# zhiyuan-yang/MILE

Hardware: AMD Instinct MI355X
Metric: MCLMC integrator particle-steps/s (integrator-steps/s x ensemble size) (higher is better)
Workload: dtype f32

## Files before the change

include/mile_hip.h:

```cpp
#ifndef MILE_HIP_H_
#define MILE_HIP_H_

#include <stdint.h>

#ifdef __cplusplus
extern "C" {
#endif

#define MILE_ABI_VERSION 6
#define MILE_MAX_LAYERS 16

typedef enum mile_status {
  MILE_OK = 0,
  MILE_ERR_INVALID = -1,
  MILE_ERR_STATE = -2,
  MILE_ERR_HIP = -3,
  MILE_ERR_NOMEM = -4
} mile_status;

typedef enum mile_activation { MILE_ACT_RELU = 0, MILE_ACT_TANH = 1, MILE_ACT_SIGMOID = 2 } mile_activation;
typedef enum mile_task { MILE_TASK_REGRESSION = 0, MILE_TASK_CLASSIFICATION = 1 } mile_task;
typedef enum mile_prior { MILE_PRIOR_NORMAL = 0, MILE_PRIOR_LAPLACE = 1 } mile_prior;
typedef enum mile_refresh { MILE_REFRESH_O_STEP_O = 0, MILE_REFRESH_STEP_O = 1 } mile_refresh;
typedef enum mile_grad_kernel {
  MILE_GRAD_AUTO = 0,
  MILE_GRAD_GENERIC = 1,
  MILE_GRAD_MFMA_W64 = 2,
  MILE_GRAD_MFMA_W128_BF16 = 3,
  MILE_GRAD_GEMM_F32 = 4,
  MILE_GRAD_LENET_F32 = 5,
  MILE_GRAD_MFMA_W64_BF16X3 = 6,
  MILE_GRAD_MFMA_WIDE_BF16X3 = 7,
  MILE_GRAD_MFMA_WIDE_BF16 = 8,
  MILE_GRAD_MFMA_NARROW_F32 = 10,
  MILE_GRAD_LENET_BF16 = 9,
  MILE_GRAD_LENETTI_F32 = 11
} mile_grad_kernel;
typedef enum mile_model { MILE_MODEL_FCN = 0, MILE_MODEL_LENET = 1, MILE_MODEL_LENETTI = 2 } mile_model;

typedef struct mile_model_spec {
  int32_t in_features;
  int32_t n_layers;
// ... 112 lines not shown

int32_t mile_set_row_window(mile_sampler *s, int64_t begin, int64_t count);

int32_t mile_warmstart_step(mile_sampler *s, float *theta, int32_t E, const mile_optim_args *args, void *stream);

int32_t mile_reserve(mile_sampler *s, int32_t E);

int32_t mile_set_grad_kernel(mile_sampler *s, int32_t which);
int32_t mile_get_grad_kernel(const mile_sampler *s);

int32_t mile_logpost_grad(mile_sampler *s, const float *theta, int32_t E, float *logp, float *grad,
                          void *stream);

int32_t mile_init(mile_sampler *s, mile_state *state, const float *noise, uint64_t seed,
                  const int32_t *particle_ids, void *stream);

int32_t mile_step(mile_sampler *s, mile_state *state, const mile_step_args *args, void *stream);

int32_t mile_tune(mile_sampler *s, mile_state *state, const mile_tune_args *args, void *stream);

int32_t mile_pointwise_loglik(mile_sampler *s, const float *theta, int32_t S, const float *X, const void *y,
                              int64_t N, float *out, void *stream);

int32_t mile_nuts_reserve(mile_sampler *s, int32_t E, int32_t max_num_doublings);

int32_t mile_nuts_step(mile_sampler *s, mile_state *state, const mile_nuts_args *a, void *stream);

int32_t mile_nuts_warmup(mile_sampler *s, mile_state *state, const mile_nuts_args *a, const mile_nuts_adapt_args *w,
                         void *stream);

int32_t mile_debug_noise(mile_sampler *s, uint64_t seed, const int32_t *particle_ids, int32_t E,
                         int64_t step, int32_t stage, float *out, void *stream);

int32_t mile_grad_launch_info(const mile_sampler *s, int32_t E, int32_t *grid_x, int32_t *grid_y,
                              int32_t *block, int32_t *lds_bytes, char *name, int32_t name_len);

int32_t mile_grad_timing_begin(mile_sampler *s);
int32_t mile_grad_timing_end(mile_sampler *s, float *total_ms, int32_t *n_launches);

#ifdef __cplusplus
}
#endif
#endif
```

mile_amd/_lib.py:

```python
from __future__ import annotations

import ctypes as C
from pathlib import Path

from mile_amd._build import LIB_PATH

MILE_MAX_LAYERS = 16
ABI_VERSION = 6

ACTIVATION_IDS = {'relu': 0, 'tanh': 1, 'sigmoid': 2}
TASK_IDS = {'regr': 0, 'regression': 0, 'classification': 1, 'class': 1}
PRIOR_IDS = {'Normal': 0, 'StandardNormal': 0, 'Laplace': 1}
REFRESH_IDS = {'O-step-O': 0, 'step-O': 1}
GRAD_KERNEL_IDS = {'auto': 0, 'generic': 1, 'mfma_w64': 2, 'mfma_w128_bf16': 3, 'gemm_f32': 4, 'lenet_f32': 5, 'mfma_w64_bf16x3': 6,
                   'mfma_wide_bf16x3': 7, 'mfma_wide_bf16': 8, 'lenet_bf16': 9, 'mfma_narrow_f32': 10,
                   'lenetti_f32': 11}


class ModelSpecC(C.Structure):
    _fields_ = [
        ('in_features', C.c_int32),
        ('n_layers', C.c_int32),
        ('widths', C.c_int32 * MILE_MAX_LAYERS),
        ('activation', C.c_int32),
        ('task', C.c_int32),
        ('prior', C.c_int32),
        ('prior_loc', C.c_float),
        ('prior_scale', C.c_float),
        ('use_bias', C.c_int32),
        ('model', C.c_int32),
        ('img_c', C.c_int32),
        ('img_h', C.c_int32),
        ('img_w', C.c_int32),
    ]


class StateC(C.Structure):
    _fields_ = [
        ('n_particles', C.c_int32),
        ('position', C.c_void_p),
        ('momentum', C.c_void_p),
# ... 50 lines not shown
        ('seed', C.c_uint64), ('particle_ids', C.c_void_p), ('step_offset', C.c_int64), ('n_steps', C.c_int32),
        ('n_thinning', C.c_int32), ('out_samples', C.c_void_p), ('out_info', C.c_void_p),
        ('out_stats', C.POINTER(C.c_int64)),
    ]


class NutsAdaptArgsC(C.Structure):
    _fields_ = [
        ('step_size', C.c_void_p), ('inverse_mass_matrix', C.c_void_p), ('da', C.c_void_p), ('welford', C.c_void_p),
        ('welford_count', C.c_void_p), ('schedule', C.POINTER(C.c_int32)), ('target_acceptance_rate', C.c_float),
    ]

SIGNATURES = {
    'mile_last_error': (C.c_char_p, []),
    'mile_abi_version': (C.c_int32, []),
    'mile_create': (C.c_int32, [C.POINTER(ModelSpecC), C.c_int32, C.POINTER(C.c_void_p)]),
    'mile_destroy': (C.c_int32, [C.c_void_p]),
    'mile_param_count': (C.c_int64, [C.c_void_p]),
    'mile_param_offsets': (C.c_int32, [C.c_void_p, C.c_int32, C.POINTER(C.c_int64), C.POINTER(C.c_int64)]),
    'mile_set_data': (C.c_int32, [C.c_void_p, C.c_void_p, C.c_void_p, C.c_int64, C.c_void_p]),
    'mile_set_row_window': (C.c_int32, [C.c_void_p, C.c_int64, C.c_int64]),
    'mile_reserve': (C.c_int32, [C.c_void_p, C.c_int32]),
    'mile_warmstart_step': (C.c_int32, [C.c_void_p, C.c_void_p, C.c_int32, C.POINTER(OptimArgsC), C.c_void_p]),
    'mile_set_grad_kernel': (C.c_int32, [C.c_void_p, C.c_int32]),
    'mile_get_grad_kernel': (C.c_int32, [C.c_void_p]),
    'mile_logpost_grad': (C.c_int32, [C.c_void_p, C.c_void_p, C.c_int32, C.c_void_p, C.c_void_p, C.c_void_p]),
    'mile_init': (C.c_int32, [C.c_void_p, C.POINTER(StateC), C.c_void_p, C.c_uint64, C.c_void_p, C.c_void_p]),
    'mile_step': (C.c_int32, [C.c_void_p, C.POINTER(StateC), C.POINTER(StepArgsC), C.c_void_p]),
    'mile_tune': (C.c_int32, [C.c_void_p, C.POINTER(StateC), C.POINTER(TuneArgsC), C.c_void_p]),
    'mile_pointwise_loglik': (C.c_int32, [C.c_void_p, C.c_void_p, C.c_int32, C.c_void_p, C.c_void_p, C.c_int64,
                                          C.c_void_p, C.c_void_p]),
    'mile_debug_noise': (C.c_int32, [C.c_void_p, C.c_uint64, C.c_void_p, C.c_int32, C.c_int64, C.c_int32,
                                     C.c_void_p, C.c_void_p]),
    'mile_grad_launch_info': (C.c_int32, [C.c_void_p, C.c_int32, C.POINTER(C.c_int32), C.POINTER(C.c_int32),
                                          C.POINTER(C.c_int32), C.POINTER(C.c_int32), C.c_char_p, C.c_int32]),
    'mile_nuts_reserve': (C.c_int32, [C.c_void_p, C.c_int32, C.c_int32]),
    'mile_nuts_step': (C.c_int32, [C.c_void_p, C.POINTER(StateC), C.POINTER(NutsArgsC), C.c_void_p]),
    'mile_nuts_warmup': (C.c_int32, [C.c_void_p, C.POINTER(StateC), C.POINTER(NutsArgsC), C.POINTER(NutsAdaptArgsC),
                                     C.c_void_p]),
    'mile_grad_timing_begin': (C.c_int32, [C.c_void_p]),
    'mile_grad_timing_end': (C.c_int32, [C.c_void_p, C.POINTER(C.c_float), C.POINTER(C.c_int32)]),
}

_lib = None


class MileHipError(RuntimeError):
    pass


def load_library(path: str | Path | None = None) -> C.CDLL:
    global _lib
    if _lib is not None and path is None:
        return _lib
    p = Path(path) if path else LIB_PATH
    if not p.exists():
        raise MileHipError(
            f'{p} not found: the MI355X HIP extension is not built. Run '
            '`python -c "import __graft_entry__ as g; g.build()"` (needs hipcc). '
            'mile_amd has no CPU fallback.')
    try:
        lib = C.CDLL(str(p))
    except OSError as exc:
        raise MileHipError(f'cannot load {p}: {exc}') from exc
    for name, (res, args) in SIGNATURES.items():
        try:
# ... 18 lines not shown
```

mile_amd/csrc/mile_hip.hip:

```cpp
#include <hip/hip_runtime.h>

#include <algorithm>
#include <cmath>
#include <cstdio>
#include <cstdlib>
#include <cstring>
#include <string>
#include <vector>

#include <dlfcn.h>

#include "mile_device.h"
#include "mile_grad_generic.h"
#include "mile_grad_narrow.h"
#include "mile_grad_w64.h"
#include "mile_grad_w128b.h"
#include "mile_grad_gemm.h"
#include "mile_mm3.h"
#include "mile_lenet.h"
#include "mile_lenet_mfma.h"
#include "mile_lenetti.h"
#include "mile_predict.h"
#include "mile_update.h"
#include "mile_nuts.h"

static thread_local std::string g_err;
static int fail(int code, const std::string &msg) { g_err = msg; return code; }
#define HIP_TRY(expr)                                                                         \
  do {                                                                                        \
    hipError_t _e = (expr);                                                                   \
    if (_e != hipSuccess)                                                                     \
      return fail(MILE_ERR_HIP, std::string(#expr) + ": " + hipGetErrorString(_e));           \
  } while (0)

static const double MCLACHLAN_B1 = 0.1931833275037836;

struct mile_sampler {
  mile_model_spec spec{};
  DevSpec ds{};
  int device = 0;
  int n_cu = 256;
  float *X = nullptr, *Xp = nullptr;
  void *Xb = nullptr, *Xt = nullptr;
  void *y = nullptr;
  int N = 0, Npad = 0, Fp = 0, Npb = 0;
  int win_begin = 0, win_count = 0;
  int E_cap = 0;
  size_t ES_cap = 0;
  float *slabs = nullptr, *llpart = nullptr, *dK = nullptr, *lold = nullptr;
  float *upart = nullptr;
  int32_t *arrive = nullptr;
  float *ev_X = nullptr, *ev_Xp = nullptr; void *ev_y = nullptr; int ev_cap = 0;
  float *alt_x = nullptr, *alt_u = nullptr, *alt_g = nullptr, *alt_logp = nullptr;
  int grad_kernel = MILE_GRAD_AUTO;
  LeNetGeom lg{};
  LeNettiGeom ng{};
  void *blas = nullptr;
  long long *dbg_buf = nullptr;
  float *tune_info = nullptr;
  float *gemm_ws = nullptr, *gemm_ones = nullptr;
  int gemm_ones_n = 0;
  size_t gemm_ws_floats = 0;
  int gemm_R = 0, gemm_E = 0;
  float *wide_ws = nullptr; size_t wide_ws_floats = 0; int wide_R = 0, wide_E = 0;
  void *wide_wt = nullptr; size_t wide_wt_bytes = 0;
  float *wide_hb = nullptr; size_t wide_hb_floats = 0;
  NutsBufs nb{};
  int nuts_E = 0, nuts_M = 0;
  int32_t *nuts_count_h = nullptr;
  bool timing = false;
  std::vector<hipEvent_t> ev;
  size_t ev_used = 0;
};

static bool w64_supported(const mile_model_spec &sp) {
  if (sp.model != MILE_MODEL_FCN) return false;
  if (sp.task != MILE_TASK_REGRESSION || sp.activation != MILE_ACT_RELU) return false;
  const int nh = sp.n_layers - 1;
  if (nh < 1 || nh > 3) return false;
  for (int l = 0; l < nh; ++l)
    if (sp.widths[l] != 64) return false;
  if (sp.widths[nh] != 2) return false;
  if (sp.in_features > 16) return false;
  return true;
// ... 256 lines not shown
  hipError_t e = hipGetDeviceCount(&cnt);
  if (e == hipSuccess && device < cnt) {
    hipDeviceProp_t prop;
    if (hipGetDeviceProperties(&prop, device) == hipSuccess) s->n_cu = prop.multiProcessorCount;
  }
  *out = s;
  return MILE_OK;
}

static void free_data(mile_sampler *s) {
  if (s->X) (void)hipFree(s->X);
  if (s->Xp) (void)hipFree(s->Xp);
  if (s->y) (void)hipFree(s->y);
  if (s->Xb) (void)hipFree(s->Xb);
  if (s->Xt) (void)hipFree(s->Xt);
  s->X = s->Xp = nullptr; s->y = nullptr; s->Xb = s->Xt = nullptr;
}
static void free_ws(mile_sampler *s) {
  if (s->slabs) (void)hipFree(s->slabs);
  if (s->llpart) (void)hipFree(s->llpart);
  if (s->dK) (void)hipFree(s->dK);
  if (s->upart) (void)hipFree(s->upart);
  s->upart = nullptr;
  if (s->lold) (void)hipFree(s->lold);
  if (s->alt_x) (void)hipFree(s->alt_x);
  if (s->alt_u) (void)hipFree(s->alt_u);
  if (s->alt_g) (void)hipFree(s->alt_g);
  if (s->alt_logp) (void)hipFree(s->alt_logp);
  s->alt_x = s->alt_u = s->alt_g = s->alt_logp = nullptr;
  if (s->tune_info) (void)hipFree(s->tune_info);
  s->tune_info = nullptr;
  if (s->arrive) (void)hipFree(s->arrive);
  s->arrive = nullptr;
  if (s->dbg_buf) (void)hipFree(s->dbg_buf);
  s->dbg_buf = nullptr;
  s->slabs = s->llpart = s->dK = s->lold = nullptr;
  s->E_cap = 0; s->ES_cap = 0;
}

static void free_nuts(mile_sampler *s) {
  NutsBufs &b = s->nb;
  float **fs[] = {&b.T, &b.Ph, &b.xe[0], &b.xe[1], &b.pe[0], &b.pe[1], &b.ge[0], &b.ge[1], &b.psT, &b.psS, &b.xs, &b.gs,
                  &b.ck_r, &b.ck_rs};
  for (float **f : fs) { if (*f) (void)hipFree(*f); *f = nullptr; }
  if (b.chain) (void)hipFree(b.chain);
  if (b.count) (void)hipFree(b.count);
  b.chain = nullptr; b.count = nullptr;
  s->nuts_E = s->nuts_M = 0;
}

int32_t mile_destroy(mile_sampler *s) {
  if (!s) return MILE_OK;
  if (s->ev_X) (void)hipFree(s->ev_X);
  if (s->ev_Xp) (void)hipFree(s->ev_Xp);
  if (s->ev_y) (void)hipFree(s->ev_y);
  free_data(s);
  free_ws(s);
  if (s->gemm_ws) (void)hipFree(s->gemm_ws);
  if (s->gemm_ones) (void)hipFree(s->gemm_ones);
  if (s->wide_ws) (void)hipFree(s->wide_ws);
  if (s->wide_wt) (void)hipFree(s->wide_wt);
  if (s->wide_hb) (void)hipFree(s->wide_hb);
  if (s->dbg_buf) (void)hipFree(s->dbg_buf);
  if (s->tune_info) (void)hipFree(s->tune_info);
  free_nuts(s);
  if (s->nuts_count_h) (void)hipHostFree(s->nuts_count_h);
// ... 62 lines not shown
    HIP_TRY(hipMalloc(&s->X, (size_t)N * F * 4));
    HIP_TRY(hipMalloc(&s->Xp, (size_t)(s->Npad + 32) * s->Fp * 4));
    HIP_TRY(hipMalloc(&s->y, (size_t)(s->Npad + 32) * 4));
  }
  HIP_TRY(hipMemsetAsync(s->Xp, 0, (size_t)(s->Npad + 32) * s->Fp * 4, st));
  HIP_TRY(hipMemcpyAsync(s->X, X, (size_t)N * F * 4, hipMemcpyDeviceToDevice, st));
  HIP_TRY(hipMemsetAsync(s->y, 0, (size_t)(s->Npad + 32) * 4, st));
  s->win_begin = s->win_count = 0;
  HIP_TRY(hipMemcpyAsync(s->y, y, (size_t)N * 4, hipMemcpyDeviceToDevice, st));
  const long long tot = (long long)s->Npad * s->Fp;
  k_pad_x<<<(unsigned)((tot + 255) / 256), 256, 0, st>>>(s->X, s->Xp, s->N, s->Npad, F, s->Fp);
  HIP_TRY(hipGetLastError());
  if (w128b_supported(s->spec)) {
    s->Npb = ((int)N + 63) / 64 * 64;
    if (!same_shape) {
      HIP_TRY(hipMalloc(&s->Xb, (size_t)s->Npb * 16 * 2));
      HIP_TRY(hipMalloc(&s->Xt, (size_t)s->Npb * 32 * 2));
    }
    const long long tb = (long long)s->Npb * 32;
    k_prep_bf16<<<(unsigned)((tb + 255) / 256), 256, 0, st>>>(s->X, (bf16 *)s->Xb, (bf16 *)s->Xt, s->N, s->Npb, F);
    HIP_TRY(hipGetLastError());
  }
  return MILE_OK;
}

int32_t mile_set_row_window(mile_sampler *s, int64_t begin, int64_t count) {
  if (!s) return fail(MILE_ERR_INVALID, "null handle");
  if (!s->X) return fail(MILE_ERR_STATE, "mile_set_row_window: call mile_set_data first");
  if (begin < 0 || count < 0 || begin + count > s->N) return fail(MILE_ERR_INVALID, "mile_set_row_window: window outside the data");
  s->win_begin = count ? (int)begin : 0;
  s->win_count = (int)count;
  return MILE_OK;
}

int32_t mile_reserve(mile_sampler *s, int32_t E) {
  if (!s || E < 1) return fail(MILE_ERR_INVALID, "mile_reserve: bad argument");
  if (!s->X) return fail(MILE_ERR_STATE, "mile_reserve: call mile_set_data first");
  HIP_TRY(hipSetDevice(s->device));
  int S = std::max(choose_S(s, E, MILE_GRAD_GENERIC), w64_supported(s->spec) ? choose_S(s, E, MILE_GRAD_MFMA_W64) : 1);
  if (w128b_supported(s->spec)) S = std::max(S, choose_S(s, E, MILE_GRAD_MFMA_W128_BF16));
  if (narrow_supported(s->spec)) S = std::max(S, choose_S(s, E, MILE_GRAD_MFMA_NARROW_F32));
  if (s->spec.model == MILE_MODEL_LENETTI) S = std::max(S, choose_S(s, E, MILE_GRAD_LENETTI_F32));
  if (E <= s->E_cap && (size_t)E * S <= s->ES_cap) return MILE_OK;
  const int En = std::max(E, s->E_cap);
  const size_t ESn = std::max((size_t)E * S, s->ES_cap);
  free_ws(s);
  HIP_TRY(hipMalloc(&s->slabs, ESn * ((s->ds.d + 3) / 4 * 4) * 4));
  HIP_TRY(hipMalloc(&s->llpart, ESn * 4));
  HIP_TRY(hipMalloc(&s->dK, (size_t)En * 4));
  HIP_TRY(hipMalloc(&s->lold, (size_t)En * 4));
  HIP_TRY(hipMalloc(&s->upart, ((size_t)En * ((s->ds.d + UPD_SEG - 1) / UPD_SEG) * UPD_NSUM + (size_t)En * 8) * 4));
  HIP_TRY(hipMalloc(&s->alt_x, (size_t)En * s->ds.d * 4));
  HIP_TRY(hipMalloc(&s->alt_u, (size_t)En * s->ds.d * 4));
  HIP_TRY(hipMalloc(&s->alt_g, (size_t)En * s->ds.d * 4));
  HIP_TRY(hipMalloc(&s->alt_logp, (size_t)En * 4));
  HIP_TRY(hipMalloc(&s->arrive, ((size_t)En * 4 + 15) / 16 * 16));
  HIP_TRY(hipMemset(s->arrive, 0, ((size_t)En * 4 + 15) / 16 * 16));
  s->E_cap = En;
  s->ES_cap = ESn;
  return MILE_OK;
}

int32_t mile_set_grad_kernel(mile_sampler *s, int32_t which) {
  if (!s) return fail(MILE_ERR_INVALID, "null handle");
  if (which < MILE_GRAD_AUTO || which > MILE_GRAD_LENETTI_F32) return fail(MILE_ERR_INVALID, "unknown grad kernel");
  if ((s->spec.model == MILE_MODEL_LENETTI) != (which == MILE_GRAD_LENETTI_F32) && which != MILE_GRAD_AUTO)
    return fail(MILE_ERR_INVALID, "LENETTI_F32 is the kernel of MILE_MODEL_LENETTI, and its only one");
  if (which == MILE_GRAD_MFMA_NARROW_F32 && !narrow_supported(s->spec))
    return fail(MILE_ERR_INVALID, "MFMA_NARROW_F32 needs an FCN with 1-3 hidden layers of width <= 64 and F <= 64 (or 4-10 of width <= 16 and F <= 16) and <= 16 outputs");
  if ((which == MILE_GRAD_MFMA_WIDE_BF16X3 || which == MILE_GRAD_MFMA_WIDE_BF16) && s->spec.model != MILE_MODEL_FCN)
    return fail(MILE_ERR_INVALID, "MFMA_WIDE_* are FCN kernels");
  if ((s->spec.model == MILE_MODEL_LENET) != (which == MILE_GRAD_LENET_F32 || which == MILE_GRAD_LENET_BF16) && which != MILE_GRAD_AUTO)
    return fail(MILE_ERR_INVALID, "LENET_F32 / LENET_BF16 are the kernels of MILE_MODEL_LENET, and its only ones");
  if (which == MILE_GRAD_LENET_BF16 && s->lg.C > 4) return fail(MILE_ERR_INVALID, "LENET_BF16 needs <= 4 image channels");
  if (which == MILE_GRAD_GEMM_F32 && !rocblas_load()) return fail(MILE_ERR_HIP, "GEMM_F32 needs librocblas.so, which could not be loaded");
  if (which == MILE_GRAD_MFMA_W128_BF16 && !w128b_supported(s->spec))
    return fail(MILE_ERR_INVALID, "MFMA_W128_BF16 needs ReLU regression with 1-3 hidden layers of width 128 and F <= 16");
  if (which == MILE_GRAD_MFMA_W64 && !w64_supported(s->spec))
    return fail(MILE_ERR_INVALID, "MFMA_W64 needs ReLU regression with 1-3 hidden layers of width 64 and F <= 16");
  if (which == MILE_GRAD_MFMA_W64_BF16X3 && !w64x3_supported(s->spec))
    return fail(MILE_ERR_INVALID, "MFMA_W64_BF16X3 needs ReLU regression with 2-3 hidden layers of width 64 and F <= 16");
  s->grad_kernel = which;
  return MILE_OK;
}
int32_t mile_get_grad_kernel(const mile_sampler *s) { return s ? resolved_kernel(s) : MILE_ERR_INVALID; }

}

static int ptr_align(const void *q) {
  const uintptr_t a = (uintptr_t)q;
  return (a & 15) == 0 ? 4 : ((a & 7) == 0 ? 2 : 1);
}

template <int AL, bool SDC>
static void launch_update_al(const UpdParams &u, int E, int nk, hipStream_t st) {
  const int nqf = u.d >> 2;
  const int nt = std::min(UPD_NT, ((nqf + nk - 1) / nk + 63) / 64 * 64);
  const int kind = SDC ? -1 : upd_kind(u);
#define MILE_UPD_CASE(NK_)                                                                       \
  if constexpr (!SDC) {                                                                          \
    if (kind == UPD_KIND_MID) { k_update_fast<NK_, AL, SDC, UPD_KIND_MID><<<E, nt, 0, st>>>(u); break; } \
    if (kind == UPD_KIND_REC) { k_update_fast<NK_, AL, SDC, UPD_KIND_REC><<<E, nt, 0, st>>>(u); break; } \
    if (kind == UPD_KIND_TUNE) {                                                                 \
      if (nt <= 768) k_update_fast<NK_, AL, SDC, UPD_KIND_TUNE, 768><<<E, nt, 0, st>>>(u);       \
      else k_update_fast<NK_, AL, SDC, UPD_KIND_TUNE><<<E, nt, 0, st>>>(u);                      \
      break;                                                                                     \
    }                                                                                            \
  }                                                                                              \
  if (nt <= 768) k_update_fast<NK_, AL, SDC, -1, 768><<<E, nt, 0, st>>>(u);                      \
  else k_update_fast<NK_, AL, SDC><<<E, nt, 0, st>>>(u);                                         \
  break;
  switch (nk) {
    case 1: MILE_UPD_CASE(1)
    case 2: MILE_UPD_CASE(2)
    case 3: MILE_UPD_CASE(3)
    default: MILE_UPD_CASE(4)
  }
#undef MILE_UPD_CASE
}

template <int AL, bool SDC>
static bool launch_update_big_al(const UpdParams &u, int E, int nk, hipStream_t st) {
  const int nqf = u.d >> 2;
  const int nt = std::min(UPD_NT, ((nqf + nk - 1) / nk + 63) / 64 * 64);
  const size_t lds = (size_t)nk * nt * 16;
#define MILE_UPD_BIG(NK_, CF_)                                                                                     \
  {                                                                                                                \
    static bool attr = false;                                                                                      \
    if (!attr) {                                                                                                   \
      if (hipFuncSetAttribute((const void *)k_update_big<NK_, AL, SDC, CF_>, hipFuncAttributeMaxDynamicSharedMemorySize, \
                              UPD_NT * NK_ * 16) != hipSuccess) return false;                                      \
      attr = true;                                                                                                 \
    }                                                                                                              \
    k_update_big<NK_, AL, SDC, CF_><<<E, nt, lds, st>>>(u);                                                        \
    return true;                                                                                                   \
  }
#define MILE_UPD_BIG_CASE(NK_) \
  case NK_:                    \
    MILE_UPD_BIG(NK_, -1)
  switch (nk) {
    MILE_UPD_BIG_CASE(5)
    MILE_UPD_BIG_CASE(6)
    MILE_UPD_BIG_CASE(7)
    MILE_UPD_BIG_CASE(8)
    MILE_UPD_BIG_CASE(9)
  }
#undef MILE_UPD_BIG_CASE
#undef MILE_UPD_BIG
  return false;
}

static bool launch_update_big(const UpdParams &u, int E, hipStream_t st) {
  const int nqf = u.d >> 2;
  const int nk = (nqf + UPD_NT - 1) / UPD_NT;
  if (nk <= UPD_QMAX || nk > UPD_QMAX_BIG || (u.flags & UPD_TUNE) || u.zA || u.zB || getenv("MILE_NO_UPD_BIG")) return false;
  int al = (u.d % 4 == 0) ? 4 : ((u.d % 2 == 0) ? 2 : 1);
  const void *ptrs[] = {u.x, u.u, u.g, u.slabs, u.sdc, u.zA, u.zB, u.out_sample, u.x_in, u.u_in, u.g_in};
  for (const void *q : ptrs)
    if (q) al = std::min(al, ptr_align(q));
  if (u.sdc) return al == 4 ? launch_update_big_al<4, true>(u, E, nk, st) : (al == 2 ? launch_update_big_al<2, true>(u, E, nk, st) : launch_update_big_al<1, true>(u, E, nk, st));
  return al == 4 ? launch_update_big_al<4, false>(u, E, nk, st) : (al == 2 ? launch_update_big_al<2, false>(u, E, nk, st) : launch_update_big_al<1, false>(u, E, nk, st));
}

static void launch_update(const UpdParams &u, int E, hipStream_t st) {
  const int nqf = u.d >> 2;
  if (nqf < 1 || nqf > UPD_NT * UPD_QMAX) {
    if (nqf >= 1 && launch_update_big(u, E, st)) return;
    if ((u.d + 3) / 4 <= UPD_NT * UPD_QMAX) { k_update<true><<<E, UPD_NT, 0, st>>>(u); return; }
    if (u.upart && getenv("MILE_NO_UPD_SEG") == nullptr) {
      const int nseg = (u.d + UPD_SEG - 1) / UPD_SEG;
      k_update_seg<1><<<dim3(nseg, E), UPD_NT, 0, st>>>(u, u.upart, nseg);
      k_update_seg<2><<<dim3(nseg, E), UPD_NT, 0, st>>>(u, u.upart, nseg);
      k_update_seg_scalars<<<(E + 255) / 256, 256, 0, st>>>(u, u.upart, nseg, E);
      return;
    }
    k_update<false><<<E, UPD_NT, 0, st>>>(u);
    return;
  }
  int al = (u.d % 4 == 0) ? 4 : ((u.d % 2 == 0) ? 2 : 1);
  const void *ptrs[] = {u.x, u.u, u.g, u.slabs, u.sdc, u.zA, u.zB, u.out_sample, u.x_in, u.u_in, u.g_in, u.t_avg, u.u_rec};
  for (const void *q : ptrs)
    if (q) al = std::min(al, ptr_align(q));
  const int nk = (nqf + UPD_NT - 1) / UPD_NT;
  if (u.sdc) {
    if (al == 4) launch_update_al<4, true>(u, E, nk, st);
    else if (al == 2) launch_update_al<2, true>(u, E, nk, st);
    else launch_update_al<1, true>(u, E, nk, st);
  } else {
    if (al == 4) launch_update_al<4, false>(u, E, nk, st);
    else if (al == 2) launch_update_al<2, false>(u, E, nk, st);
    else launch_update_al<1, false>(u, E, nk, st);
  }
}

hipError_t mile_launch_w64_split_fq2(int nh, const GradParams &gp, int E, hipStream_t st);

template <int NH, int FQ, bool SPLIT = false>
static hipError_t launch_w64(const GradParams &gp, const W64Fuse &fz, int E, hipStream_t st) {
  using LY = W64Layout<NH, FQ, SPLIT>;
  static bool attr_set = false;
  if (!attr_set) {
    hipError_t e = hipFuncSetAttribute((const void *)k_grad_w64<NH, FQ, SPLIT>, hipFuncAttributeMaxDynamicSharedMemorySize, LY::BYTES);
    if (e != hipSuccess) return e;
    attr_set = true;
  }
  if constexpr (W64FuseArg<FQ, SPLIT>::FUSABLE) {
    k_grad_w64<NH, FQ, SPLIT><<<dim3(gp.S, E), 256, LY::BYTES, st>>>(gp, fz);
  } else {
    if (fz.enabled) return hipErrorInvalidValue;
    k_grad_w64<NH, FQ, SPLIT><<<dim3(gp.S, E), 256, LY::BYTES, st>>>(gp, W64NoFuse{0});
  }
  return hipGetLastError();
}
// ... 1115 lines not shown
  if (!state->position || !state->momentum || !state->logdensity || !state->logdensity_grad)
    return fail(MILE_ERR_INVALID, "mile_step: null state field");
  if (!a->step_size || !a->L) return fail(MILE_ERR_INVALID, "mile_step: step_size and L are required");
  if (a->n_steps < 0) return fail(MILE_ERR_INVALID, "mile_step: n_steps < 0");
  if (a->refresh != MILE_REFRESH_O_STEP_O && a->refresh != MILE_REFRESH_STEP_O)
    return fail(MILE_ERR_INVALID, "mile_step: unknown refresh mode");
  const int E = state->n_particles, d = s->ds.d;
  if (E < 1) return fail(MILE_ERR_INVALID, "mile_step: n_particles must be >= 1");
  if (a->n_steps == 0) return MILE_OK;
  hipStream_t st = (hipStream_t)stream;
  HIP_TRY(hipSetDevice(s->device));
  const int kernel = resolved_kernel(s);
  const int S = choose_S(s, E, kernel);
  if (!s->X) return fail(MILE_ERR_STATE, "no data: call mile_set_data first");
  if (E > s->E_cap || (size_t)E * S > s->ES_cap) return fail(MILE_ERR_STATE, "workspace too small: call mile_reserve(E) first");

  UpdParams up{};
  up.d = d; up.E = E; up.S = S; up.dp = (d + 3) / 4 * 4;
  up.prior = s->ds.prior; up.prior_loc = s->ds.prior_loc; up.prior_scale = s->ds.prior_scale;
  up.x = state->position; up.u = state->momentum; up.g = state->logdensity_grad; up.logp = state->logdensity;
  up.slabs = s->slabs; up.llpart = s->llpart;
  up.eps = a->step_size; up.L = a->L; up.sdc = a->sqrt_diag_cov;
  up.seed = a->seed; up.pids = a->particle_ids;
  up.dK = s->dK; up.lold = s->lold; up.upart = s->upart;
  const float b1 = (float)MCLACHLAN_B1, b2 = (float)(1.0 - 2.0 * MCLACHLAN_B1);
  const bool oso = a->refresh == MILE_REFRESH_O_STEP_O;
  const size_t Ed = (size_t)E * d;
  auto noise_at = [&](int i, int k) -> const float * { return a->noise ? a->noise + ((size_t)i * 2 + k) * Ed : nullptr; };

  UpdParams probe = up;
  probe.zA = a->noise; probe.zB = a->noise; probe.out_sample = a->out_samples;
  const bool fused = fuse_ok(s, kernel, probe);
  if (fused) HIP_TRY(hipMemsetAsync(s->arrive, 0, ((size_t)E * 4 + 15) / 16 * 16, st));
  int kept = 0;
  for (int i = 0; i < a->n_steps; ++i) {
    const int64_t gstep = a->step_offset + i;
    if (i == 0) {
      UpdParams u = up;
      u.flags = UPD_START | UPD_B2 | UPD_A | (oso ? UPD_OB : 0);
      u.zB = noise_at(i, 0); u.stepB = (uint32_t)gstep; u.stageB = 0; u.hB = 0.5f;
      u.coef_b2 = b1; u.coef_a = 0.5f;
      launch_update(u, E, st);
    }
    {
      UpdParams u = up;
      u.flags = UPD_FROM_SLABS | UPD_B1 | UPD_A | UPD_NO_G;
      u.coef_b1 = b2; u.coef_a = 0.5f;
      const int rc = grad_then_update(s, state->position, E, u, fused, st);
      if (rc) return rc;
    }
    {
      UpdParams u = up;
      const bool last = (i == a->n_steps - 1);
      u.flags = UPD_FROM_SLABS | UPD_B1 | UPD_OA | UPD_RECORD;
      u.coef_b1 = b1;
      u.zA = noise_at(i, 1); u.stepA = (uint32_t)gstep; u.stageA = 1; u.hA = oso ? 0.5f : 1.0f;
      if (!last) {
        u.flags |= UPD_B2 | UPD_A | (oso ? UPD_OB : 0) | UPD_NO_G;
        u.zB = noise_at(i + 1, 0); u.stepB = (uint32_t)(gstep + 1); u.stageB = 0; u.hB = 0.5f;
        u.coef_b2 = b1; u.coef_a = 0.5f;
      }
      if (a->out_info) u.out_info = a->out_info + (size_t)i * E * 3;
      if (a->out_samples && a->n_thinning > 0 && (gstep % a->n_thinning) == 0) {
        u.out_sample = a->out_samples + (size_t)kept * Ed;
        ++kept;
      }
      const int rc = grad_then_update(s, state->position, E, u, fused, st);
      if (rc) return rc;
    }
  }
  HIP_TRY(hipGetLastError());
  return MILE_OK;
}

int32_t mile_tune(mile_sampler *s, mile_state *state, const mile_tune_args *a, void *stream) {
  if (!s || !state || !a) return fail(MILE_ERR_INVALID, "mile_tune: null argument");
  if (!state->position || !state->momentum || !state->logdensity || !state->logdensity_grad)
    return fail(MILE_ERR_INVALID, "mile_tune: null state field");
  if (!a->step_size || !a->L || !a->step_size_max || !a->time || !a->x_average || !a->stream_weight || !a->stream_average)
    return fail(MILE_ERR_INVALID, "mile_tune: null tuner array");
  if (a->n_steps < 0 || a->schedule_total < 1) return fail(MILE_ERR_INVALID, "mile_tune: bad step counts");
  if (a->refresh != MILE_REFRESH_O_STEP_O && a->refresh != MILE_REFRESH_STEP_O)
    return fail(MILE_ERR_INVALID, "mile_tune: unknown refresh mode");
  const int E = state->n_particles, d = s->ds.d;
  if (E < 1) return fail(MILE_ERR_INVALID, "mile_tune: n_particles must be >= 1");
  if ((d >> 2) < 1) return fail(MILE_ERR_INVALID, "mile_tune: d < 4");
  const bool big = (d >> 2) > UPD_NT * UPD_QMAX || getenv("MILE_TUNE_POST") != nullptr;
  if (a->n_steps == 0) return MILE_OK;
  hipStream_t st = (hipStream_t)stream;
  HIP_TRY(hipSetDevice(s->device));
  if (!s->X) return fail(MILE_ERR_STATE, "no data: call mile_set_data first");
  const int S = choose_S(s, E, resolved_kernel(s));
  if (E > s->E_cap || (size_t)E * S > s->ES_cap) return fail(MILE_ERR_STATE, "workspace too small: call mile_reserve(E) first");

  struct Buf { float *x, *u, *g, *logp; };
  const Buf A{state->position, state->momentum, state->logdensity_grad, state->logdensity};
  const Buf B{s->alt_x, s->alt_u, s->alt_g, s->alt_logp};
  UpdParams up{};
  up.d = d; up.E = E; up.S = S; up.dp = (d + 3) / 4 * 4;
  up.prior = s->ds.prior; up.prior_loc = s->ds.prior_loc; up.prior_scale = s->ds.prior_scale;
// ... 111 lines not shown
      if (a->out_info) u.out_info = a->out_info + (size_t)i * E * 3;
      if (i + 1 < a->n_steps && !no_merge) {
        u.flags |= UPD_B2 | UPD_A | (oso ? UPD_OB : 0);
        u.zB = noise_at(i + 1, 0); u.stepB = (uint32_t)(gstep + 1); u.stageB = 0; u.hB = 0.5f;
        u.coef_b2 = b1; u.coef_a = 0.5f;
        u.x_in = nxt.x; u.u_in = nxt.u;
        u.x_acc = nxt.x; u.u_rec = nxt.u;
        u.x = cur.x; u.u = cur.u;
        u.force_restart = getenv("MILE_TUNE_FORCE_RESTART") != nullptr;
      }
      const int rc = grad_then_update(s, nxt.x, E, u, fused, st);
      if (rc) return rc;
    }
  }
  if (a->n_steps & 1) {
    HIP_TRY(hipMemcpyAsync(A.x, B.x, Ed * 4, hipMemcpyDeviceToDevice, st));
    HIP_TRY(hipMemcpyAsync(A.u, B.u, Ed * 4, hipMemcpyDeviceToDevice, st));
    HIP_TRY(hipMemcpyAsync(A.g, B.g, Ed * 4, hipMemcpyDeviceToDevice, st));
    HIP_TRY(hipMemcpyAsync(A.logp, B.logp, (size_t)E * 4, hipMemcpyDeviceToDevice, st));
  }
  HIP_TRY(hipGetLastError());
  return MILE_OK;
}

int32_t mile_debug_noise(mile_sampler *s, uint64_t seed, const int32_t *particle_ids, int32_t E,
                         int64_t step, int32_t stage, float *out, void *stream) {
  if (!s || !out || E < 1) return fail(MILE_ERR_INVALID, "mile_debug_noise: bad argument");
  HIP_TRY(hipSetDevice(s->device));
  k_debug_noise<<<E, AUX_NT, 0, (hipStream_t)stream>>>(s->ds.d, seed, particle_ids, (uint32_t)step, (uint32_t)stage, out);
  HIP_TRY(hipGetLastError());
  return MILE_OK;
}

int32_t mile_nuts_reserve(mile_sampler *s, int32_t E, int32_t max_num_doublings) {
  if (!s || E < 1 || max_num_doublings < 1 || max_num_doublings > NUTS_MAX_DOUBLINGS)
    return fail(MILE_ERR_INVALID, "mile_nuts_reserve: E >= 1 and 1 <= max_num_doublings <= 12");
  const int rc = mile_reserve(s, E);
  if (rc) return rc;
  if (E <= s->nuts_E && max_num_doublings <= s->nuts_M) return MILE_OK;
  const int En = std::max(E, s->nuts_E), Mn = std::max(max_num_doublings, s->nuts_M);
  free_nuts(s);
  const size_t Ed = (size_t)En * s->ds.d * 4;
  NutsBufs &b = s->nb;
  float **fs[] = {&b.T, &b.Ph, &b.xe[0], &b.xe[1], &b.pe[0], &b.pe[1], &b.ge[0], &b.ge[1], &b.psT, &b.psS, &b.xs, &b.gs};
  for (float **f : fs) HIP_TRY(hipMalloc(f, Ed));
  HIP_TRY(hipMalloc(&b.ck_r, Ed * Mn));
  HIP_TRY(hipMalloc(&b.ck_rs, Ed * Mn));
  HIP_TRY(hipMalloc(&b.chain, (size_t)En * sizeof(NutsChain)));
  HIP_TRY(hipMalloc(&b.count, 16));
  HIP_TRY(hipMemset(b.T, 0, Ed));
  if (!s->nuts_count_h) HIP_TRY(hipHostMalloc((void **)&s->nuts_count_h, 16, hipHostMallocDefault));
  s->nuts_E = En; s->nuts_M = Mn;
  return MILE_OK;
}

static int nuts_run(mile_sampler *s, mile_state *state, const mile_nuts_args *a, const mile_nuts_adapt_args *w, void *stream) {
  const char *fn = w ? "mile_nuts_warmup" : "mile_nuts_step";
  if (!s || !state || !a) return fail(MILE_ERR_INVALID, std::string(fn) + ": null argument");
  if (!state->position || !state->logdensity || !state->logdensity_grad) return fail(MILE_ERR_INVALID, std::string(fn) + ": null state field");
  const int E = state->n_particles, d = s->ds.d, M = a->max_num_doublings;
  if (E < 1 || a->n_steps < 0) return fail(MILE_ERR_INVALID, std::string(fn) + ": n_particles >= 1 and n_steps >= 0");
  if (M < 1 || M > NUTS_MAX_DOUBLINGS) return fail(MILE_ERR_INVALID, std::string(fn) + ": 1 <= max_num_doublings <= 12");
  if (w) {
    if (!w->step_size || !w->inverse_mass_matrix || !w->da || !w->welford || !w->welford_count || !w->schedule)
      return fail(MILE_ERR_INVALID, "mile_nuts_warmup: null adaptation field");
  } else if (!a->step_size || !a->inverse_mass_matrix) {
// ... 75 lines not shown
```

mile_amd/csrc/mile_update.h:

```cpp
#pragma once
#include <cstdlib>

#include "mile_device.h"

enum : int32_t {
  UPD_FROM_SLABS = 1 << 0,
  UPD_START = 1 << 1,
  UPD_B1 = 1 << 2,
  UPD_OA = 1 << 3,
  UPD_RECORD = 1 << 4,
  UPD_OB = 1 << 5,
  UPD_B2 = 1 << 6,
  UPD_A = 1 << 7,
  UPD_TUNE = 1 << 8,
  UPD_NO_G = 1 << 9,
};

struct UpdParams {
  int32_t d, E, S, flags;
  int32_t dp;
  int32_t prior;
  float prior_loc, prior_scale;
  float *x, *u, *g, *logp;
  const float *slabs, *llpart;
  const float *eps, *L, *sdc;
  const float *zA, *zB;
  uint64_t seed;
  const int32_t *pids;
  uint32_t stepA, stageA, stepB, stageB;
  float coef_b1, coef_b2, coef_a;
  float hA, hB;
  float *dK, *lold;
  float *out_sample;
  float *out_info;
  const float *x_in, *u_in, *g_in, *logp_in;
  float *t_eps;
  float *t_eps_max, *t_time, *t_xavg;
  float *t_W;
  float *t_avg;
  const float *bk_x, *bk_u, *bk_g, *bk_logp;
  float t_mask;
  float t_var;
  float t_trust, t_decay;
  float *upart;
  float *u_rec;
  float *x_acc;
  int32_t force_restart;
};

struct Chain {
  float M[4][4];
  float c[4];
  __device__ __forceinline__ float norm() const {
    float s = 0.0f;
#pragma unroll
    for (int a = 0; a < 4; ++a)
#pragma unroll
      for (int b = 0; b < 4; ++b) s = fmaf(c[a] * M[a][b], c[b], s);
    return sqrtf(s);
  }
  __device__ __forceinline__ float B(float eps, float coef, float gnorm, int d) {
    float ue = 0.0f;
#pragma unroll
    for (int a = 0; a < 4; ++a) ue = fmaf(c[a], M[a][1], ue);
    const float delta = eps * coef * gnorm / (float)(d - 1);
    const float omz = -expm1f(-delta);
    const float zeta = 1.0f - omz;
    const float beta = omz * (1.0f + zeta + ue * omz);
#pragma unroll
    for (int a = 0; a < 4; ++a) c[a] *= 2.0f * zeta;
    c[1] += beta;
    const float n = norm();
    if (n > 1e-13f)
#pragma unroll
      for (int a = 0; a < 4; ++a) c[a] /= n;
    return (float)(d - 1) * (delta + log1pf(0.5f * (1.0f - ue) * expm1f(-2.0f * delta)));
  }
  __device__ __forceinline__ void O(int k, float hstep, float L, int d) {
    const float nu = sqrtf(expm1f(2.0f * hstep / L) / (float)d);
    c[k] += nu;
// ... 726 lines not shown
      }
    }
    if constexpr (BIG) __builtin_amdgcn_sched_barrier(0);
  }
  if (has_tail) {
    if (t_acc) {
      float *a0 = p.t_avg + (size_t)e * 2 * d + 4 * (size_t)nqf + tid, *a1 = a0 + d;
      *a0 = (t_Wold * *a0 + t_wgt * tx) * t_den;
      *a1 = (t_Wold * *a1 + t_wgt * tx * tx) * t_den;
    }
    float v = tu;
    if (merged) p.u_rec[to] = nan_to_num(fmaf(rc0, tu, fmaf(rc1, tg, rc2 * ta)));
    if (!merged || simple) {
      if (any_op) { v = fmaf(c0, tu, fmaf(c1, tg, fmaf(c2, ta, c3 * tb))); if (tune && !merged) v = nan_to_num(v); p.u[to] = v; }
      if (p.out_sample) p.out_sample[to] = tx;
      if (doA) p.x[to] = fmaf(ea * tsd, v, tx);
    }
  }
  return merged && !simple;
}

template <int NK, int AL, bool SDC>
__device__ __forceinline__ void upd_tune_restart(const UpdParams &p, const int e, const int tid, const int nt,
                                                 float (*red)[UPD_NSUM + 1], float *bc) {
  __syncthreads();
  UpdParams q = p;
  q.flags = UPD_START | UPD_B2 | UPD_A | (p.flags & UPD_OB);
  q.x_in = p.x_acc; q.u_in = p.u_rec; q.g_in = p.g; q.logp_in = p.logp;
  q.eps = p.t_eps;
  q.u_rec = nullptr; q.x_acc = nullptr; q.out_info = nullptr; q.out_sample = nullptr; q.zA = nullptr;
  upd_fast_body<NK, AL, SDC, false, -1>(q, e, tid, nt, red, bc);
}

template <int NK, int AL, bool SDC, int CF = -1, int MAXT = UPD_NT>
static __global__ __launch_bounds__(MAXT) void k_update_fast(const UpdParams p) {
  __shared__ float red[UPD_NW][UPD_NSUM + 1];
  __shared__ float bc[16];
  const bool again = upd_fast_body<NK, AL, SDC, false, CF>(p, blockIdx.x, threadIdx.x, blockDim.x, red, bc);
  if constexpr (CF < 0 || (CF & UPD_TUNE) != 0) {
    if (again) upd_tune_restart<NK, AL, SDC>(p, blockIdx.x, threadIdx.x, blockDim.x, red, bc);
  }
}

#define UPD_QMAX_BIG 9
template <int NK, int AL, bool SDC, int CF = -1>
static __global__ __launch_bounds__(UPD_NT) void k_update_big(const UpdParams p) {
  __shared__ float red[UPD_NW][UPD_NSUM + 1];
  __shared__ float bc[16];
  extern __shared__ __attribute__((aligned(16))) char upd_gl[];
  upd_fast_body<NK, AL, SDC, false, CF, true>(p, blockIdx.x, threadIdx.x, blockDim.x, red, bc, nullptr, reinterpret_cast<f32x4 *>(upd_gl));
}

static inline int upd_kind(const UpdParams &u) {
  if (u.prior != MILE_PRIOR_NORMAL || u.sdc || getenv("MILE_NO_UPD_KIND")) return -1;
  if (u.flags == UPD_KIND_MID) return UPD_KIND_MID;
  if (u.flags == UPD_KIND_REC) return UPD_KIND_REC;
  if (u.flags == UPD_KIND_TUNE && u.u_rec) return UPD_KIND_TUNE;
  return -1;
}

#define AUX_NT 256
__device__ __forceinline__ float slab_grad_logprior(const float *sl, int S, int dp, int i, int prior, float loc, float scale,
                                                    float theta_i, float &pv) {
  float gi = 0.0f;
  for (int s = 0; s < S; ++s) gi += sl[(size_t)s * dp + i];
  const float t = (theta_i - loc) / scale;
  if (prior == MILE_PRIOR_NORMAL) { gi -= t / scale; pv += -0.5f * t * t; }
  else { gi -= (t > 0.0f ? 1.0f : (t < 0.0f ? -1.0f : 0.0f)) / scale; pv += -fabsf(t); }
  return gi;
}
__device__ __forceinline__ double llpart_logprior(const float *llpart, int S, int e, int d, int prior, float scale, double pv) {
  double t = pv;
  for (int s = 0; s < S; ++s) t += (double)llpart[(size_t)e * S + s];
  t += prior == MILE_PRIOR_NORMAL ? -(double)d * (log((double)scale) + 0.91893853320467274)
                                  : -(double)d * log(2.0 * (double)scale);
  return t;
}

static __global__ __launch_bounds__(AUX_NT) void k_finalize(int d, int dp, int S, int prior, float loc, float scale,
                                                     const float *theta, const float *slabs,
                                                     const float *llpart, float *grad, float *logp) {
  __shared__ float red[AUX_NT / 64];
  const int tid = threadIdx.x, e = blockIdx.x;
  const size_t base = (size_t)e * d;
  const float *sl = slabs + (size_t)e * S * dp;
  float pv = 0.0f;
  for (int i = tid; i < d; i += AUX_NT) grad[base + i] = slab_grad_logprior(sl, S, dp, i, prior, loc, scale, theta[base + i], pv);
  pv = wave_sum(pv);
  if ((tid & 63) == 0) red[tid >> 6] = pv;
  __syncthreads();
  if (tid == 0) {
    double t = 0.0;
// ... 161 lines not shown
```

mile_amd/engine.py:

```python
from __future__ import annotations

import ctypes as C
import math
from typing import NamedTuple

import torch

from mile_amd import _lib
from mile_amd.spec import IMAGE_SPECS, LeNetSpec, LeNettiSpec, ModelSpec


class IntegratorState(NamedTuple):

    position: torch.Tensor
    momentum: torch.Tensor
    logdensity: torch.Tensor
    logdensity_grad: torch.Tensor


class MCLMCInfo(NamedTuple):

    logdensity: torch.Tensor
    kinetic_change: torch.Tensor
    energy_change: torch.Tensor
# ... 396 lines not shown
        sc = _lib.StateC()
        sc.n_particles = E
        sc.position, sc.logdensity, sc.logdensity_grad = (state.position.data_ptr(), state.logdensity.data_ptr(),
                                                          state.logdensity_grad.data_ptr())
        if n_steps:
            with torch.cuda.device(self.device):
                _lib.check(self.lib.mile_nuts_warmup(self._h, C.byref(sc), C.byref(a), C.byref(w), self._stream()), self.lib)
        return self._nuts_info(info), samples

    def pointwise_loglik(self, theta, X, y) -> torch.Tensor:
        theta = _f32(theta, self.device, name='theta')
        lead = theta.shape[:-1]
        th = theta.reshape(-1, self.d).contiguous()
        X = _f32(X, self.device, name='X')
        y = torch.as_tensor(y, device=self.device)
        y = (y.to(torch.float32) if self.spec.task == 'regr' else y.to(torch.int32)).contiguous()
        if isinstance(self.spec, IMAGE_SPECS) and X.ndim == 4:
            X = X.reshape(X.shape[0], -1).contiguous()
        if X.ndim != 2 or X.shape[1] != self.spec.in_features or y.shape != (X.shape[0],):
            raise ValueError('X must be [N, F] and y [N]')
        if self.spec.task != 'regr' and y.numel():
            if int(y.min()) < 0 or int(y.max()) >= self.spec.hidden_structure[-1]:
                raise ValueError('class labels out of range')
        out = torch.empty((th.shape[0], X.shape[0]), dtype=torch.float32, device=self.device)
        with torch.cuda.device(self.device):
            _lib.check(self.lib.mile_pointwise_loglik(self._h, _ptr(th), th.shape[0], _ptr(X), _ptr(y), X.shape[0],
                                                      _ptr(out), self._stream()), self.lib)
        return out.reshape(*lead, X.shape[0])

    @property
    def supports_device_tuner(self) -> bool:
        return self.d >= 4

    def debug_noise(self, seed: int, E: int, step: int, stage: int, particle_ids=None):
        ids = self._ids(particle_ids, E)
        out = torch.empty((E, self.d), dtype=torch.float32, device=self.device)
        with torch.cuda.device(self.device):
            _lib.check(self.lib.mile_debug_noise(self._h, C.c_uint64(seed), _ptr(ids), E, step, stage, _ptr(out),
                                                 self._stream()), self.lib)
        return out
```

Baseline: 913,300.

## Prefill Philox noise in extra workgroups of the mid update kernel

When no external noise is supplied and the fused path is off, the mid-step update kernel now launches twice as many workgroups, and the extra ones generate the Philox normal noise needed by the following record update into a device buffer. The record update then reads that precomputed noise instead of generating it inline. This moves RNG work off the critical record kernel into otherwise idle parallel workgroups. The cost is extra global-memory writes and reads of the noise buffer, plus a lazily allocated scratch buffer of two E×d floats.

```diff
diff --git a/include/mile_hip.h b/include/mile_hip.h
--- a/include/mile_hip.h
+++ b/include/mile_hip.h
@@ -7,7 +7,7 @@
 extern "C" {
 #endif
 
-#define MILE_ABI_VERSION 6
+#define MILE_ABI_VERSION 7
 #define MILE_MAX_LAYERS 16
 
 typedef enum mile_status {
@@ -186,6 +186,8 @@
 int32_t mile_debug_noise(mile_sampler *s, uint64_t seed, const int32_t *particle_ids, int32_t E,
                          int64_t step, int32_t stage, float *out, void *stream);
 
+int64_t mile_debug_prefill_count(const mile_sampler *s);
+
 int32_t mile_grad_launch_info(const mile_sampler *s, int32_t E, int32_t *grid_x, int32_t *grid_y,
                               int32_t *block, int32_t *lds_bytes, char *name, int32_t name_len);
 
diff --git a/mile_amd/_lib.py b/mile_amd/_lib.py
--- a/mile_amd/_lib.py
+++ b/mile_amd/_lib.py
@@ -6,7 +6,7 @@
 from mile_amd._build import LIB_PATH
 
 MILE_MAX_LAYERS = 16
-ABI_VERSION = 6
+ABI_VERSION = 7
 
 ACTIVATION_IDS = {'relu': 0, 'tanh': 1, 'sigmoid': 2}
 TASK_IDS = {'regr': 0, 'regression': 0, 'classification': 1, 'class': 1}
@@ -123,6 +123,7 @@
                                           C.c_void_p, C.c_void_p]),
     'mile_debug_noise': (C.c_int32, [C.c_void_p, C.c_uint64, C.c_void_p, C.c_int32, C.c_int64, C.c_int32,
                                      C.c_void_p, C.c_void_p]),
+    'mile_debug_prefill_count': (C.c_int64, [C.c_void_p]),
     'mile_grad_launch_info': (C.c_int32, [C.c_void_p, C.c_int32, C.POINTER(C.c_int32), C.POINTER(C.c_int32),
                                           C.POINTER(C.c_int32), C.POINTER(C.c_int32), C.c_char_p, C.c_int32]),
     'mile_nuts_reserve': (C.c_int32, [C.c_void_p, C.c_int32, C.c_int32]),
diff --git a/mile_amd/csrc/mile_hip.hip b/mile_amd/csrc/mile_hip.hip
--- a/mile_amd/csrc/mile_hip.hip
+++ b/mile_amd/csrc/mile_hip.hip
@@ -50,6 +50,9 @@
   float *slabs = nullptr, *llpart = nullptr, *dK = nullptr, *lold = nullptr;
   float *upart = nullptr;
   int32_t *arrive = nullptr;
+  float *nzbuf = nullptr;
+  int nz_E = 0;
+  int64_t nz_launches = 0;
   float *ev_X = nullptr, *ev_Xp = nullptr; void *ev_y = nullptr; int ev_cap = 0;
   float *alt_x = nullptr, *alt_u = nullptr, *alt_g = nullptr, *alt_logp = nullptr;
   int grad_kernel = MILE_GRAD_AUTO;
@@ -372,6 +375,9 @@
   s->tune_info = nullptr;
   if (s->arrive) (void)hipFree(s->arrive);
   s->arrive = nullptr;
+  if (s->nzbuf) (void)hipFree(s->nzbuf);
+  s->nzbuf = nullptr;
+  s->nz_E = 0;
   if (s->dbg_buf) (void)hipFree(s->dbg_buf);
   s->dbg_buf = nullptr;
   s->slabs = s->llpart = s->dK = s->lold = nullptr;
@@ -500,6 +506,8 @@
   s->win_count = (int)count;
   return MILE_OK;
 }
+
+static size_t nz_stride(int E, int d) { return ((size_t)E * d + 3) / 4 * 4; }
 
 int32_t mile_reserve(mile_sampler *s, int32_t E) {
   if (!s || E < 1) return fail(MILE_ERR_INVALID, "mile_reserve: bad argument");
@@ -565,9 +573,10 @@
   const int nqf = u.d >> 2;
   const int nt = std::min(UPD_NT, ((nqf + nk - 1) / nk + 63) / 64 * 64);
   const int kind = SDC ? -1 : upd_kind(u);
+  const int nwg_mid = (u.nz_A || u.nz_B) ? 2 * E : E;
 #define MILE_UPD_CASE(NK_)                                                                       \
   if constexpr (!SDC) {                                                                          \
-    if (kind == UPD_KIND_MID) { k_update_fast<NK_, AL, SDC, UPD_KIND_MID><<<E, nt, 0, st>>>(u); break; } \
+    if (kind == UPD_KIND_MID) { k_update_fast<NK_, AL, SDC, UPD_KIND_MID><<<nwg_mid, nt, 0, st>>>(u); break; } \
     if (kind == UPD_KIND_REC) { k_update_fast<NK_, AL, SDC, UPD_KIND_REC><<<E, nt, 0, st>>>(u); break; } \
     if (kind == UPD_KIND_TUNE) {                                                                 \
       if (nt <= 768) k_update_fast<NK_, AL, SDC, UPD_KIND_TUNE, 768><<<E, nt, 0, st>>>(u);       \
@@ -630,9 +639,13 @@
   return al == 4 ? launch_update_big_al<4, false>(u, E, nk, st) : (al == 2 ? launch_update_big_al<2, false>(u, E, nk, st) : launch_update_big_al<1, false>(u, E, nk, st));
 }
 
+static bool update_prefills(const UpdParams &u) {
+  return upd_fast_d(u.d) && !u.sdc && upd_kind(u) == UPD_KIND_MID;
+}
+
 static void launch_update(const UpdParams &u, int E, hipStream_t st) {
   const int nqf = u.d >> 2;
-  if (nqf < 1 || nqf > UPD_NT * UPD_QMAX) {
+  if (!upd_fast_d(u.d)) {
     if (nqf >= 1 && launch_update_big(u, E, st)) return;
     if ((u.d + 3) / 4 <= UPD_NT * UPD_QMAX) { k_update<true><<<E, UPD_NT, 0, st>>>(u); return; }
     if (u.upart && getenv("MILE_NO_UPD_SEG") == nullptr) {
@@ -646,7 +659,7 @@
     return;
   }
   int al = (u.d % 4 == 0) ? 4 : ((u.d % 2 == 0) ? 2 : 1);
-  const void *ptrs[] = {u.x, u.u, u.g, u.slabs, u.sdc, u.zA, u.zB, u.out_sample, u.x_in, u.u_in, u.g_in, u.t_avg, u.u_rec};
+  const void *ptrs[] = {u.x, u.u, u.g, u.slabs, u.sdc, u.zA, u.zB, u.out_sample, u.x_in, u.u_in, u.g_in, u.t_avg, u.u_rec, u.nz_A, u.nz_B};
   for (const void *q : ptrs)
     if (q) al = std::min(al, ptr_align(q));
   const int nk = (nqf + UPD_NT - 1) / UPD_NT;
@@ -1828,6 +1841,15 @@
   probe.zA = a->noise; probe.zB = a->noise; probe.out_sample = a->out_samples;
   const bool fused = fuse_ok(s, kernel, probe);
   if (fused) HIP_TRY(hipMemsetAsync(s->arrive, 0, ((size_t)E * 4 + 15) / 16 * 16, st));
+  const char *dv = getenv("MILE_DEBUG");
+  const bool prefill = !fused && !a->noise && upd_fast_d(d) && !(dv && (atoi(dv) & 128));
+  if (prefill && s->nz_E < E) {
+    if (s->nzbuf) HIP_TRY(hipFree(s->nzbuf));
+    s->nzbuf = nullptr;
+    s->nz_E = 0;
+    HIP_TRY(hipMalloc(&s->nzbuf, 2 * nz_stride(s->E_cap, d) * 4));
+    s->nz_E = s->E_cap;
+  }
   int kept = 0;
   for (int i = 0; i < a->n_steps; ++i) {
     const int64_t gstep = a->step_offset + i;
@@ -1838,30 +1860,43 @@
       u.coef_b2 = b1; u.coef_a = 0.5f;
       launch_update(u, E, st);
     }
+    UpdParams ur = up;
+    {
+      const bool last = (i == a->n_steps - 1);
+      ur.flags = UPD_FROM_SLABS | UPD_B1 | UPD_OA | UPD_RECORD;
+      ur.coef_b1 = b1;
+      ur.zA = noise_at(i, 1); ur.stepA = (uint32_t)gstep; ur.stageA = 1; ur.hA = oso ? 0.5f : 1.0f;
+      if (!last) {
+        ur.flags |= UPD_B2 | UPD_A | (oso ? UPD_OB : 0) | UPD_NO_G;
+        ur.zB = noise_at(i + 1, 0); ur.stepB = (uint32_t)(gstep + 1); ur.stageB = 0; ur.hB = 0.5f;
+        ur.coef_b2 = b1; ur.coef_a = 0.5f;
+      }
+      if (a->out_info) ur.out_info = a->out_info + (size_t)i * E * 3;
+      if (a->out_samples && a->n_thinning > 0 && (gstep % a->n_thinning) == 0) {
+        ur.out_sample = a->out_samples + (size_t)kept * Ed;
+        ++kept;
+      }
+    }
     {
       UpdParams u = up;
       u.flags = UPD_FROM_SLABS | UPD_B1 | UPD_A | UPD_NO_G;
       u.coef_b1 = b2; u.coef_a = 0.5f;
+      if (prefill && update_prefills(u)) {
+        ++s->nz_launches;
+        if (!ur.zA) {
+          u.nz_A = s->nzbuf; u.nz_stepA = ur.stepA; u.nz_stageA = ur.stageA;
+          ur.zA = u.nz_A;
+        }
+        if ((ur.flags & UPD_OB) && !ur.zB) {
+          u.nz_B = s->nzbuf + nz_stride(s->nz_E, d); u.nz_stepB = ur.stepB; u.nz_stageB = ur.stageB;
+          ur.zB = u.nz_B;
+        }
+      }
       const int rc = grad_then_update(s, state->position, E, u, fused, st);
       if (rc) return rc;
     }
     {
-      UpdParams u = up;
-      const bool last = (i == a->n_steps - 1);
-      u.flags = UPD_FROM_SLABS | UPD_B1 | UPD_OA | UPD_RECORD;
-      u.coef_b1 = b1;
-      u.zA = noise_at(i, 1); u.stepA = (uint32_t)gstep; u.stageA = 1; u.hA = oso ? 0.5f : 1.0f;
-      if (!last) {
-        u.flags |= UPD_B2 | UPD_A | (oso ? UPD_OB : 0) | UPD_NO_G;
-        u.zB = noise_at(i + 1, 0); u.stepB = (uint32_t)(gstep + 1); u.stageB = 0; u.hB = 0.5f;
-        u.coef_b2 = b1; u.coef_a = 0.5f;
-      }
-      if (a->out_info) u.out_info = a->out_info + (size_t)i * E * 3;
-      if (a->out_samples && a->n_thinning > 0 && (gstep % a->n_thinning) == 0) {
-        u.out_sample = a->out_samples + (size_t)kept * Ed;
-        ++kept;
-      }
-      const int rc = grad_then_update(s, state->position, E, u, fused, st);
+      const int rc = grad_then_update(s, state->position, E, ur, fused, st);
       if (rc) return rc;
     }
   }
@@ -2039,6 +2074,8 @@
   return MILE_OK;
 }
 
+int64_t mile_debug_prefill_count(const mile_sampler *s) { return s ? s->nz_launches : -1; }
+
 int32_t mile_nuts_reserve(mile_sampler *s, int32_t E, int32_t max_num_doublings) {
   if (!s || E < 1 || max_num_doublings < 1 || max_num_doublings > NUTS_MAX_DOUBLINGS)
     return fail(MILE_ERR_INVALID, "mile_nuts_reserve: E >= 1 and 1 <= max_num_doublings <= 12");
diff --git a/mile_amd/csrc/mile_update.h b/mile_amd/csrc/mile_update.h
--- a/mile_amd/csrc/mile_update.h
+++ b/mile_amd/csrc/mile_update.h
@@ -46,6 +46,8 @@
   float *u_rec;
   float *x_acc;
   int32_t force_restart;
+  float *nz_A, *nz_B;
+  uint32_t nz_stepA, nz_stageA, nz_stepB, nz_stageB;
 };
 
 struct Chain {
@@ -838,10 +840,42 @@
   upd_fast_body<NK, AL, SDC, false, -1>(q, e, tid, nt, red, bc);
 }
 
+template <int NK, int AL>
+__device__ __forceinline__ void upd_noise_body(const UpdParams &p, const int e, const int tid, const int nt) {
+  const int d = p.d, nqf = d >> 2, ntail = d & 3;
+  const size_t base = (size_t)e * d;
+  const uint32_t pid = p.pids ? (uint32_t)p.pids[e] : (uint32_t)e;
+#pragma unroll
+  for (int k = 0; k < NK; ++k) {
+    const int q = tid + k * nt;
+    if (q < nqf) {
+      if (p.nz_A) st4<AL>(p.nz_A + base + 4 * (size_t)q, philox_normal4(q, pid, p.nz_stepA, p.nz_stageA, p.seed));
+      if (p.nz_B) st4<AL>(p.nz_B + base + 4 * (size_t)q, philox_normal4(q, pid, p.nz_stepB, p.nz_stageB, p.seed));
+    }
+  }
+  if (ntail && tid == 0) {
+    const size_t o = base + 4 * (size_t)nqf;
+    if (p.nz_A) {
+      const f32x4 z = philox_normal4(nqf, pid, p.nz_stepA, p.nz_stageA, p.seed);
+      for (int t = 0; t < ntail; ++t) p.nz_A[o + t] = z[t];
+    }
+    if (p.nz_B) {
+      const f32x4 z = philox_normal4(nqf, pid, p.nz_stepB, p.nz_stageB, p.seed);
+      for (int t = 0; t < ntail; ++t) p.nz_B[o + t] = z[t];
+    }
+  }
+}
+
 template <int NK, int AL, bool SDC, int CF = -1, int MAXT = UPD_NT>
 static __global__ __launch_bounds__(MAXT) void k_update_fast(const UpdParams p) {
   __shared__ float red[UPD_NW][UPD_NSUM + 1];
   __shared__ float bc[16];
+  if constexpr (CF == UPD_KIND_MID) {
+    if ((int)blockIdx.x >= p.E) {
+      upd_noise_body<NK, AL>(p, blockIdx.x - p.E, threadIdx.x, blockDim.x);
+      return;
+    }
+  }
   const bool again = upd_fast_body<NK, AL, SDC, false, CF>(p, blockIdx.x, threadIdx.x, blockDim.x, red, bc);
   if constexpr (CF < 0 || (CF & UPD_TUNE) != 0) {
     if (again) upd_tune_restart<NK, AL, SDC>(p, blockIdx.x, threadIdx.x, blockDim.x, red, bc);
@@ -864,6 +898,8 @@
   if (u.flags == UPD_KIND_TUNE && u.u_rec) return UPD_KIND_TUNE;
   return -1;
 }
+
+static inline bool upd_fast_d(int d) { return (d >> 2) >= 1 && (d >> 2) <= UPD_NT * UPD_QMAX; }
 
 #define AUX_NT 256
 __device__ __forceinline__ float slab_grad_logprior(const float *sl, int S, int dp, int i, int prior, float loc, float scale,
diff --git a/mile_amd/engine.py b/mile_amd/engine.py
--- a/mile_amd/engine.py
+++ b/mile_amd/engine.py
@@ -452,6 +452,9 @@
     def supports_device_tuner(self) -> bool:
         return self.d >= 4
 
+    def debug_prefill_count(self) -> int:
+        return int(self.lib.mile_debug_prefill_count(self._h))
+
     def debug_noise(self, seed: int, E: int, step: int, stage: int, particle_ids=None):
         ids = self._ids(particle_ids, E)
         out = torch.empty((E, self.d), dtype=torch.float32, device=self.device)
```

Result: faster. 931,300 (median of 6 runs) (+2.0%).
